# graphdeco-inria/reduced-3dgs

Measured on NVIDIA H100. Metric: rendered Mpixels/s fwd+bwd, higher is better.
Workload: dtype f32

## Files before the change

reduced-3dgs_b200/csrc/gsb_render.cu:

```cuda
#include <cstddef>
#include <cstdlib>
#include "gsb_common.cuh"

namespace gsb {

__device__ __forceinline__ void red_add_v4(float* addr, float a, float b, float c, float d)
{
	asm volatile("red.global.add.v4.f32 [%0], {%1, %2, %3, %4};" ::"l"(addr), "f"(a), "f"(b), "f"(c), "f"(d) : "memory");
}

#define SREC_BYTES 48
__device__ __forceinline__ float4 lds128(uint32_t addr)
{
	float4 v;
	asm volatile("ld.shared.v4.f32 {%0, %1, %2, %3}, [%4];" : "=f"(v.x), "=f"(v.y), "=f"(v.z), "=f"(v.w) : "r"(addr));
	return v;
}
__device__ __forceinline__ float2 lds64(uint32_t addr)
{
	float2 v;
	asm volatile("ld.shared.v2.f32 {%0, %1}, [%2];" : "=f"(v.x), "=f"(v.y) : "r"(addr));
	return v;
}

#define STATS_FIXED_SCALE 68719476736.0f
template <bool STATS, bool MAPS, bool FIXED = false>
__global__ void __launch_bounds__(256, 6) render_forward_kernel(const uint2* __restrict__ ranges,
	const uint32_t* __restrict__ point_list,
	int W, int H, const float4* __restrict__ rec, const float* __restrict__ bg,
	float* __restrict__ final_T, uint32_t* __restrict__ n_contrib, float* __restrict__ out_color, uint32_t* __restrict__ tile_max,
	int32_t* __restrict__ touched_pixels, float* __restrict__ transmittance, float* __restrict__ out_invdepth, float* __restrict__ out_alpha)
{
	__shared__ __align__(16) float4 s_rec[256 * 3];
	__shared__ uint32_t s_id[STATS ? 256 : 1];
	__shared__ uint32_t s_max;
	const int tid = threadIdx.x, lane = tid & 31, warp = tid >> 5;
	const int tile = blockIdx.y * gridDim.x + blockIdx.x;
	const int wx0 = blockIdx.x * GSB_TILE_X + (warp & 1) * 8, wy0 = blockIdx.y * GSB_TILE_Y + (warp >> 1) * 4;
	const int px = wx0 + (lane & 7), py = wy0 + (lane >> 3);
	const bool inside = px < W && py < H;
	const float pxf = (float)px, pyf = (float)py;
	const float rx0 = (float)wx0, rx1 = (float)(wx0 + 7), ry0 = (float)wy0, ry1 = (float)(wy0 + 3);
	const uint2 range = ranges[tile];
	uint32_t sbase = (uint32_t)__cvta_generic_to_shared(s_rec);
	asm volatile("" : "+r"(sbase));
	if (tid == 0) s_max = 0;

	uint32_t Tb = inside ? 0x3f800000u : 0xbf800000u;
	float C0 = 0.0f, C1 = 0.0f, C2 = 0.0f, D = 0.0f;
	uint32_t last = 0;
	for (uint32_t b = range.x; b < range.y; b += 256)
	{
		if (__syncthreads_count((int)Tb < 0) == 256) break;
		const int n = min(256u, range.y - b);
		if (tid < n)
		{
			const uint32_t id = point_list[b + tid];
			const float4 r0 = rec[3 * (size_t)id], r1 = rec[3 * (size_t)id + 1], r2 = rec[3 * (size_t)id + 2];
			s_rec[3 * tid] = r0; s_rec[3 * tid + 1] = r1;
			s_rec[3 * tid + 2] = MAPS ? make_float4(r2.x, r2.y, __fdiv_rn(1.0f, r2.z), r2.w) : r2;
			if (STATS) s_id[tid] = id;
		}
		__syncthreads();
		bool warp_done = __all_sync(0xffffffffu, (int)Tb < 0);
		for (int c0 = 0; c0 < n && !warp_done; c0 += 32)
		{
			const int j = c0 + lane;
			bool keep = false;
			if (j < n)
			{
				const float4 r0 = lds128(sbase + j * SREC_BYTES), r1 = lds128(sbase + j * SREC_BYTES + 16);
				keep = rect_may_contribute(r1.x, r1.y, r0.x, r0.y, r0.z, r0.w, rx0, rx1, ry0, ry1);
			}
			unsigned mask = __ballot_sync(0xffffffffu, keep);
			const uint32_t cbase = sbase + c0 * SREC_BYTES;
			uint32_t nbase = (b - range.x) + c0 + 1;
			asm volatile("" : "+r"(nbase));
			while (mask)
			{
				const int bit = __ffs(mask) - 1; mask &= mask - 1;
				const uint32_t addr = cbase + bit * SREC_BYTES;
				const float4 r0 = lds128(addr), r1 = lds128(addr + 16);
				float2 gb; float invd = 0.0f;
				if (MAPS) { const float4 r2 = lds128(addr + 32); gb = make_float2(r2.x, r2.y); invd = r2.z; }
				else gb = lds64(addr + 32);
				const float T = __uint_as_float(Tb);
				const float dx = __fsub_rn(r1.x, pxf), dy = __fsub_rn(r1.y, pyf);
				const float power = pair_power(r0.x, r0.y, r0.z, dx, dy);
				const bool inwin = !(power > 0.0f) && !(power < r0.w);
				const float alpha = fminf(0.99f, __fmul_rn(r1.z, exp_loop(power)));
				const bool cand = inwin && !(alpha < 1.0f / 255.0f);
				const float test_T = __fmul_rn(T, __fsub_rn(1.0f, alpha));
				const bool stop = cand && (test_T < 0.0001f);
				const bool v = cand && !(test_T < 0.0001f);
				if (STATS)
				{
					const unsigned cm = __ballot_sync(0xffffffffu, v);
					if (cm)
					{
						float ts = v ? T : 0.0f;
#pragma unroll
						for (int o = 16; o > 0; o >>= 1) ts += __shfl_xor_sync(0xffffffffu, ts, o);
						if (lane == 0)
						{
							const uint32_t gid = s_id[c0 + bit];
							atomicAdd(&touched_pixels[gid], (int)__popc(cm));
							if (FIXED) atomicAdd(reinterpret_cast<unsigned long long*>(transmittance) + gid, __float2ull_rn(ts * STATS_FIXED_SCALE));
							else atomicAdd(&transmittance[gid], ts);
						}
					}
				}
				if (v)
				{
					C0 = __fmaf_rn(T, __fmul_rn(r1.w, alpha), C0);
					C1 = __fmaf_rn(T, __fmul_rn(gb.x, alpha), C1);
					C2 = __fmaf_rn(T, __fmul_rn(gb.y, alpha), C2);
					if (MAPS) D = __fmaf_rn(T, __fmul_rn(invd, alpha), D);
					Tb = __float_as_uint(test_T);
					last = nbase + bit;
				}
				if (stop) Tb |= 0x80000000u;
			}
			warp_done = __all_sync(0xffffffffu, (int)Tb < 0);
		}
	}
	const float T = __uint_as_float(Tb & 0x7fffffffu);
	if (inside)
	{
		const size_t pid = (size_t)W * py + px, N = (size_t)W * H;
		final_T[pid] = T;
		n_contrib[pid] = last;
		out_color[pid] = __fmaf_rn(bg[0], T, C0);
		out_color[N + pid] = __fmaf_rn(bg[1], T, C1);
		out_color[2 * N + pid] = __fmaf_rn(bg[2], T, C2);
		if (MAPS) { out_invdepth[pid] = D; out_alpha[pid] = __fsub_rn(1.0f, T); }
	}
	uint32_t m = inside ? last : 0u;
#pragma unroll
	for (int o = 16; o > 0; o >>= 1) m = max(m, __shfl_xor_sync(0xffffffffu, m, o));
	__syncthreads();
	if (lane == 0 && m) atomicMax(&s_max, m);
	__syncthreads();
	if (tid == 0) tile_max[tile] = s_max;
}

#define BWD_BATCH 64
#define STASH_LD 36
#define ACC_STRIDE 9

__device__ __forceinline__ void mma_tf32(float (&d)[4], uint32_t a0, uint32_t a1, uint32_t a2, uint32_t a3, uint32_t b0, uint32_t b1)
{
	asm volatile("mma.sync.aligned.m16n8k8.row.col.f32.tf32.tf32.f32 {%0,%1,%2,%3}, {%4,%5,%6,%7}, {%8,%9}, {%0,%1,%2,%3};"
		: "+f"(d[0]), "+f"(d[1]), "+f"(d[2]), "+f"(d[3]) : "r"(a0), "r"(a1), "r"(a2), "r"(a3), "r"(b0), "r"(b1));
}
__device__ __forceinline__ void split_tf32(float v, uint32_t& hi, uint32_t& lo)
{
	hi = __float_as_uint(v) & 0xffffe000u;
	lo = __float_as_uint(v - __uint_as_float(hi));
}

__device__ __forceinline__ float rcp_approx(float x)
{
	float r;
	asm("rcp.approx.ftz.f32 %0, %1;" : "=f"(r) : "f"(x));
	return r;
}
__device__ __forceinline__ void cp_async16(uint32_t smem_addr, const void* gptr)
{
	asm volatile("cp.async.ca.shared.global [%0], [%1], 16;" ::"r"(smem_addr), "l"(gptr) : "memory");
}
__device__ __forceinline__ void cp_async_commit() { asm volatile("cp.async.commit_group;" ::: "memory"); }
__device__ __forceinline__ void cp_async_wait_all() { asm volatile("cp.async.wait_group 0;" ::: "memory"); }

#define BWD_STAGES 4
template <int NCH> struct BwdWarp {
	float w[16 * STASH_LD];
	float u[16 * STASH_LD];
	float dlp[NCH * 32];
	uint32_t rowid[16];
	uint8_t queue[BWD_BATCH + 16];
};
#define BW_OFF_U (16 * STASH_LD * 4)
#define BW_OFF_ROWID(NCH) (2 * 16 * STASH_LD * 4 + (NCH) * 32 * 4)
#define BW_OFF_QUEUE(NCH) (BW_OFF_ROWID(NCH) + 16 * 4)
template <int NCH> struct BwdSmem {
	float4 rec[BWD_STAGES][BWD_BATCH * 3];
	uint64_t full[BWD_STAGES];
	uint64_t empty[BWD_STAGES];
	float wgt[8 * 32];
	BwdWarp<NCH> wp[8];
};
static_assert(offsetof(BwdWarp<3>, u) == BW_OFF_U && offsetof(BwdWarp<3>, rowid) == BW_OFF_ROWID(3) && offsetof(BwdWarp<3>, queue) == BW_OFF_QUEUE(3), "BwdWarp layout");
static_assert(offsetof(BwdWarp<4>, u) == BW_OFF_U && offsetof(BwdWarp<4>, rowid) == BW_OFF_ROWID(4) && offsetof(BwdWarp<4>, queue) == BW_OFF_QUEUE(4), "BwdWarp layout");
static_assert(sizeof(BwdWarp<3>) % 16 == 0 && sizeof(BwdWarp<4>) % 16 == 0, "BwdWarp alignment");

__device__ __forceinline__ void red_add_v2(float* addr, float a, float b)
{
	asm volatile("red.global.add.v2.f32 [%0], {%1, %2};" ::"l"(addr), "f"(a), "f"(b) : "memory");
}


#define DET_NS(MAPS) ((MAPS) ? 10 : 9)
template <bool MAPS, bool DET = false>
__global__ void __launch_bounds__(256, DET ? 3 : 4) render_backward_kernel(const uint2* __restrict__ ranges,
	const uint32_t* __restrict__ point_list,
	int W, int H, const float4* __restrict__ rec, const float* __restrict__ bg,
	const float* __restrict__ final_Ts, const uint32_t* __restrict__ n_contrib, const uint32_t* __restrict__ tile_max,
	const float* __restrict__ dL_dpixels, float* __restrict__ acc, const float* __restrict__ dL_dinvdepth, const float* __restrict__ dL_dalpha,
	float* __restrict__ parts = nullptr, const uint32_t* __restrict__ slot_offset = nullptr, const uint2* __restrict__ rect = nullptr,
	unsigned long long num_slots = 0)
{
	constexpr int NCH = MAPS ? 4 : 3;
	constexpr int NS = DET_NS(MAPS);
	extern __shared__ __align__(16) unsigned char s_dyn_raw[];
	BwdSmem<NCH>& S = *reinterpret_cast<BwdSmem<NCH>*>(s_dyn_raw);
	float* const ebuf = reinterpret_cast<float*>(s_dyn_raw + sizeof(BwdSmem<NCH>));
	const int tid = threadIdx.x, lane = tid & 31, warp = tid >> 5;
	const int tile = blockIdx.y * gridDim.x + blockIdx.x;
	const uint32_t hi = tile_max[tile];
	if (hi == 0) return;
	const int lx = (warp & 1) * 8 + (lane & 7), ly = (warp >> 1) * 4 + (lane >> 3);
	const int tx0 = blockIdx.x * GSB_TILE_X, ty0 = blockIdx.y * GSB_TILE_Y;
	const int px = tx0 + lx, py = ty0 + ly;
	const bool inside = px < W && py < H;
	const float pxf = (float)px, pyf = (float)py;
	const float rx0 = (float)(tx0 + (warp & 1) * 8), rx1 = rx0 + 7.0f, ry0 = (float)(ty0 + (warp >> 1) * 4), ry1 = ry0 + 3.0f;
	const uint2 range = ranges[tile];
	const size_t pid = (size_t)W * py + px, N = (size_t)W * H;
	uint32_t sbase0 = (uint32_t)__cvta_generic_to_shared(&S.rec[0][0]);
	asm volatile("" : "+r"(sbase0));
	BwdWarp<NCH>& Wp = S.wp[warp];
	uint32_t wbase = (uint32_t)__cvta_generic_to_shared(&Wp);
	asm volatile("" : "+r"(wbase));
	const unsigned lt_mask = (1u << lane) - 1u;

	const float T_final = inside ? final_Ts[pid] : 0.0f;
	float T = T_final;
	const uint32_t last_contributor = inside ? n_contrib[pid] : 0u;
	float dLp0 = 0.f, dLp1 = 0.f, dLp2 = 0.f;
	if (inside) { dLp0 = dL_dpixels[pid]; dLp1 = dL_dpixels[N + pid]; dLp2 = dL_dpixels[2 * N + pid]; }
	float bg_dot_dpixel = bg[0] * dLp0 + bg[1] * dLp1 + bg[2] * dLp2;
	float dLd = 0.f, ar3 = 0.f, lc3 = 0.f;
	if (MAPS && inside)
	{
		if (dL_dinvdepth) dLd = dL_dinvdepth[pid];
		if (dL_dalpha) bg_dot_dpixel -= dL_dalpha[pid];
	}
	float ar0 = 0.f, ar1 = 0.f, ar2 = 0.f, lc0 = 0.f, lc1 = 0.f, lc2 = 0.f, last_alpha = 0.f;
	uint32_t wmax = last_contributor;
#pragma unroll
	for (int o = 16; o > 0; o >>= 1) wmax = max(wmax, __shfl_xor_sync(0xffffffffu, wmax, o));

	const int fg = lane >> 2, ft = lane & 3;
	float* sw = Wp.w;
	float* su = Wp.u;
	uint32_t nrows = 0;
	int buf = 0;

	if (tid < 32)
	{
		const float qx = (float)(tid & 7) - 3.5f, qy = (float)(tid >> 3) - 1.5f;
		S.wgt[0 * 32 + tid] = 1.0f; S.wgt[1 * 32 + tid] = qx; S.wgt[2 * 32 + tid] = qy;
		S.wgt[3 * 32 + tid] = qx * qx; S.wgt[4 * 32 + tid] = qx * qy; S.wgt[5 * 32 + tid] = qy * qy;
		S.wgt[6 * 32 + tid] = 0.0f; S.wgt[7 * 32 + tid] = 0.0f;
	}
	Wp.dlp[lane] = dLp0; Wp.dlp[32 + lane] = dLp1; Wp.dlp[64 + lane] = dLp2;
	if (MAPS) Wp.dlp[96 + lane] = dLd;
	const float cxw = rx0 + 3.5f, cyw = ry0 + 1.5f;
	if (DET) for (int i = tid; i < 8 * BWD_BATCH * NS; i += 256) ebuf[i] = 0.0f;
	__syncthreads();

	auto flush_rows = [&]() {
		if (nrows == 0) return;
		for (uint32_t r = nrows; r < 16; r++) { sw[r * STASH_LD + lane] = 0.f; su[r * STASH_LD + lane] = 0.f; }
		__syncwarp();
		if (!DET && ft == 0)
		{
			if (fg < nrows) asm volatile("prefetch.global.L1 [%0];" ::"l"(rec + 3 * (size_t)Wp.rowid[fg]));
			if (fg + 8 < nrows) asm volatile("prefetch.global.L1 [%0];" ::"l"(rec + 3 * (size_t)Wp.rowid[fg + 8]));
		}
		float dw[4] = { 0.f, 0.f, 0.f, 0.f }, du[4] = { 0.f, 0.f, 0.f, 0.f };
		const float* dl = Wp.dlp + (fg < NCH ? fg : 0) * 32;
#pragma unroll
		for (int kk = 0; kk < 4; kk++)
		{
			const int c0 = 8 * kk + ft, c1 = c0 + 4;
			const uint32_t bw0 = __float_as_uint(S.wgt[fg * 32 + c0]), bw1 = __float_as_uint(S.wgt[fg * 32 + c1]);
			uint32_t buh0, buh1, bul0, bul1;
			split_tf32(fg < NCH ? dl[c0] : 0.0f, buh0, bul0);
			split_tf32(fg < NCH ? dl[c1] : 0.0f, buh1, bul1);
			uint32_t h0, h1, h2, h3, l0, l1, l2, l3;
			split_tf32(sw[fg * STASH_LD + c0], h0, l0); split_tf32(sw[(fg + 8) * STASH_LD + c0], h1, l1);
			split_tf32(sw[fg * STASH_LD + c1], h2, l2); split_tf32(sw[(fg + 8) * STASH_LD + c1], h3, l3);
			mma_tf32(dw, h0, h1, h2, h3, bw0, bw1);
			mma_tf32(dw, l0, l1, l2, l3, bw0, bw1);
			split_tf32(su[fg * STASH_LD + c0], h0, l0); split_tf32(su[(fg + 8) * STASH_LD + c0], h1, l1);
			split_tf32(su[fg * STASH_LD + c1], h2, l2); split_tf32(su[(fg + 8) * STASH_LD + c1], h3, l3);
			mma_tf32(du, h0, h1, h2, h3, buh0, buh1);
			mma_tf32(du, l0, l1, l2, l3, buh0, buh1);
			mma_tf32(du, h0, h1, h2, h3, bul0, bul1);
		}
		const int q1 = (lane & ~3) | 1, q2 = (lane & ~3) | 2;
#pragma unroll
		for (int h = 0; h < 2; h++)
		{
			const float My = __shfl_sync(0xffffffffu, dw[2 * h], q1), Mxx = __shfl_sync(0xffffffffu, dw[2 * h + 1], q1);
			const float Mxy = __shfl_sync(0xffffffffu, dw[2 * h], q2), Myy = __shfl_sync(0xffffffffu, dw[2 * h + 1], q2);
			const float c2 = __shfl_sync(0xffffffffu, du[2 * h], q1);
			float dinvd = 0.f;
			if (MAPS) dinvd = __shfl_sync(0xffffffffu, du[2 * h + 1], q1);
			const uint32_t row = fg + 8 * h;
			if (ft == 0 && row < nrows)
			{
				const uint32_t gid = Wp.rowid[row];
				float4 r0, r1;
				if (DET)
				{
					const uint32_t ra = sbase0 + (uint32_t)(buf * BWD_BATCH * 3) * 16u + gid * SREC_BYTES;
					r0 = lds128(ra); r1 = lds128(ra + 16);
				}
				else { r0 = __ldg(rec + 3 * (size_t)gid); r1 = __ldg(rec + 3 * (size_t)gid + 1); }
				const float X = r1.x - cxw, Y = r1.y - cyw, o = r1.z;
				const float M0 = dw[2 * h], Mx = dw[2 * h + 1];
				const float Sx = X * M0 - Mx, Sy = Y * M0 - My;
				const float Sxx = X * X * M0 - 2.0f * X * Mx + Mxx;
				const float Sxy = X * Y * M0 - X * My - Y * Mx + Mxy;
				const float Syy = Y * Y * M0 - 2.0f * Y * My + Myy;
				if (DET)
				{
					float* e = ebuf + (warp * BWD_BATCH + gid) * NS;
					e[0] = du[2 * h]; e[1] = du[2 * h + 1]; e[2] = c2; e[3] = M0;
					e[4] = -o * (r0.x * Sx + r0.y * Sy); e[5] = -o * (r0.z * Sy + r0.y * Sx); e[6] = o * Sxx; e[7] = o * Sxy;
					e[8] = o * Syy;
					if (MAPS) e[9] = dinvd;
					continue;
				}
				float* a = acc + 12 * (size_t)gid;
				red_add_v4(a, du[2 * h], du[2 * h + 1], c2, M0);
				red_add_v4(a + 4, -o * (r0.x * Sx + r0.y * Sy), -o * (r0.z * Sy + r0.y * Sx), o * Sxx, o * Sxy);
				if (MAPS) red_add_v2(a + 8, o * Syy, dinvd);
				else atomicAdd(a + 8, o * Syy);
			}
		}
		__syncwarp();
		nrows = 0;
	};

	auto list_id = [&](uint32_t bi) -> uint32_t {
		const uint32_t k = bi * BWD_BATCH + tid;
		return (tid < BWD_BATCH && k < hi) ? point_list[range.x + (hi - 1 - k)] : 0xffffffffu;
	};
	auto issue = [&](uint32_t bi, uint32_t id) {
		const int st = bi % BWD_STAGES;
		if (id != 0xffffffffu)
		{
			mbar_arrive_expect_tx(&S.full[st], 48u);
			tma_bulk_g2s(&S.rec[st][3 * tid], rec + 3 * (size_t)id, 48u, &S.full[st]);
		}
		else mbar_arrive(&S.full[st]);
	};
	const uint32_t nb = (hi + BWD_BATCH - 1) / BWD_BATCH;
	if (tid == 0)
	{
		for (int k = 0; k < BWD_STAGES; k++) { mbar_init(&S.full[k], BWD_BATCH); mbar_init(&S.empty[k], 8); }
		mbar_fence_init();
	}
	__syncthreads();
	uint32_t id_next = 0xffffffffu;
	if (tid < BWD_BATCH)
	{
		for (uint32_t k = 0; k < BWD_STAGES - 1 && k < nb; k++) issue(k, list_id(k));
		id_next = list_id(BWD_STAGES - 1);
	}
	for (uint32_t bi = 0; bi < nb; bi++)
	{
		const uint32_t b = bi * BWD_BATCH;
		const int n = min((uint32_t)BWD_BATCH, hi - b);
		buf = bi % BWD_STAGES;
		if (tid < BWD_BATCH && bi + BWD_STAGES - 1 < nb)
		{
			if (bi >= 1) mbar_wait(&S.empty[(bi - 1) % BWD_STAGES], ((bi - 1) / BWD_STAGES) & 1u);
			issue(bi + BWD_STAGES - 1, id_next);
			id_next = list_id(bi + BWD_STAGES);
		}
		mbar_wait(&S.full[buf], (bi / BWD_STAGES) & 1u);
		const uint32_t sbase = sbase0 + (uint32_t)(buf * BWD_BATCH * 3) * 16u;
		uint32_t qn = 0;
		for (int c0 = 0; c0 < n; c0 += 32)
		{
			const int j = c0 + lane;
			bool keep = false;
			if (j < n && (hi - 1 - b - j) < wmax)
			{
				const float4 r0 = lds128(sbase + j * SREC_BYTES), r1 = lds128(sbase + j * SREC_BYTES + 16);
				keep = rect_may_contribute(r1.x, r1.y, r0.x, r0.y, r0.z, r0.w, rx0, rx1, ry0, ry1);
			}
			const unsigned mask = __ballot_sync(0xffffffffu, keep);
			if (keep) Wp.queue[qn + __popc(mask & lt_mask)] = (uint8_t)j;
			qn += __popc(mask);
		}
		__syncwarp();
		uint32_t posb = hi - 1 - b;
		asm volatile("" : "+r"(posb));
		uint32_t jj = 0, jnext;
		if (qn) asm volatile("ld.shared.u8 %0, [%1+%2];" : "=r"(jj) : "r"(wbase), "n"(BW_OFF_QUEUE(NCH)));
		for (uint32_t q = 0; q < qn; q++, jj = jnext)
		{
			asm volatile("ld.shared.u8 %0, [%1+%2];" : "=r"(jnext) : "r"(wbase + q), "n"(BW_OFF_QUEUE(NCH) + 1));
			const uint32_t pos = posb - jj;
			const uint32_t addr = sbase + jj * SREC_BYTES;
			const float4 r0 = lds128(addr), r1 = lds128(addr + 16);
			const float dx = __fsub_rn(r1.x, pxf), dy = __fsub_rn(r1.y, pyf);
			const float power = pair_power(r0.x, r0.y, r0.z, dx, dy);
			const float G = exp_loop(power);
			const float alpha = fminf(0.99f, __fmul_rn(r1.z, G));
			const bool active = (pos < last_contributor) && !(power > 0.0f) && !(power < r0.w) && !(alpha < 1.0f / 255.0f);
			if (!__any_sync(0xffffffffu, active)) continue;
			float wv = 0.f, uv = 0.f;
			const float4 r2 = lds128(addr + 32);
			if (active)
			{
				const float inv = rcp_approx(1.0f - alpha);
				T = T * inv;
				uv = alpha * T;
				const float cr = r1.w, cg = r2.x, cb = r2.y;
				const float oml = 1.0f - last_alpha;
				ar0 = last_alpha * lc0 + oml * ar0; lc0 = cr;
				ar1 = last_alpha * lc1 + oml * ar1; lc1 = cg;
				ar2 = last_alpha * lc2 + oml * ar2; lc2 = cb;
				float dL_dalpha = (cr - ar0) * dLp0 + (cg - ar1) * dLp1 + (cb - ar2) * dLp2;
				if (MAPS)
				{
					const float invd = rcp_approx(r2.z);
					float dLd_p;
					asm volatile("ld.shared.f32 %0, [%1+%2];" : "=f"(dLd_p) : "r"(wbase + lane * 4), "n"(2 * 16 * STASH_LD * 4 + 96 * 4));
					ar3 = last_alpha * lc3 + oml * ar3; lc3 = invd;
					dL_dalpha += (invd - ar3) * dLd_p;
				}
				dL_dalpha *= T;
				last_alpha = alpha;
				dL_dalpha += (-T_final * inv) * bg_dot_dpixel;
				wv = G * dL_dalpha;
			}
			{
				const uint32_t sa = wbase + (nrows * STASH_LD + lane) * 4;
				asm volatile("st.shared.f32 [%0], %1;" ::"r"(sa), "f"(wv) : "memory");
				asm volatile("st.shared.f32 [%0+%2], %1;" ::"r"(sa), "f"(uv), "n"(BW_OFF_U) : "memory");
				if (lane == 0) asm volatile("st.shared.f32 [%0+%2], %1;" ::"r"(wbase + nrows * 4), "f"(DET ? __uint_as_float(jj) : r2.w), "n"(BW_OFF_ROWID(NCH)) : "memory");
			}
			nrows++;
			if (nrows == 16) flush_rows();
		}
		if (DET)
		{
			flush_rows();
			__syncthreads();
			const int j = tid >> 2;
			if (j < n)
			{
				const uint32_t gid = __float_as_uint(S.rec[buf][3 * j + 2].w);
				const uint2 rc = rect[gid];
				const uint32_t minx = rc.x & 0xffffu, maxx = rc.x >> 16, miny = rc.y & 0xffffu;
				const unsigned long long slot = (unsigned long long)slot_offset[gid] + (blockIdx.y - miny) * (maxx - minx) + (blockIdx.x - minx);
				for (int k = tid & 3; k < NS; k += 4)
				{
					float s = ebuf[j * NS + k];
					ebuf[j * NS + k] = 0.0f;
#pragma unroll
					for (int w = 1; w < 8; w++)
					{
						s += ebuf[(w * BWD_BATCH + j) * NS + k];
						ebuf[(w * BWD_BATCH + j) * NS + k] = 0.0f;
					}
					if (slot < num_slots) parts[slot * NS + k] = s;
				}
			}
			__syncthreads();
		}
		__syncwarp();
		if (lane == 0) mbar_arrive(&S.empty[buf]);
	}
	flush_rows();
}

__global__ void __launch_bounds__(256) stats_fixed_to_float_kernel(int P, const unsigned long long* __restrict__ fixed, float* __restrict__ out)
{
	const int i = blockIdx.x * blockDim.x + threadIdx.x;
	if (i < P) out[i] = __fmul_rn(__ull2float_rn(fixed[i]), 1.0f / STATS_FIXED_SCALE);
}

int launch_stats_fixed_to_float(int P, const unsigned long long* fixed, float* out, cudaStream_t stream)
{
	if (P <= 0) return GSB_OK;
	ProfScope prof(K_TOOLS, stream);
	stats_fixed_to_float_kernel<<<(P + 255) / 256, 256, 0, stream>>>(P, fixed, out);
	GSB_LAUNCHED();
	GSB_CUDA_OK(cudaGetLastError());
	return GSB_OK;
}

int launch_render_forward(const ForwardRequest& req, const ImageState& img, const BinningState& b, const GeomState& g)
{
	const int W = req.cam->width, H = req.cam->height;
	const dim3 grid((W + GSB_TILE_X - 1) / GSB_TILE_X, (H + GSB_TILE_Y - 1) / GSB_TILE_Y);
	const bool fixed = req.touched_pixels && req.transmittance_fixed;
	const bool stats = fixed || (req.touched_pixels && req.transmittance);
	const bool maps = !stats && req.out_invdepth && req.out_alpha;
	float* const transmittance = fixed ? reinterpret_cast<float*>(req.transmittance_fixed) : req.transmittance;
	ProfScope prof(K_RENDER_FWD, req.stream);
	return dispatch([&](auto stats, auto maps, auto fixed) -> int {
		if constexpr (!(stats && maps) && (stats || !fixed))
			render_forward_kernel<stats, maps, fixed><<<grid, 256, 0, req.stream>>>(img.ranges, b.point_list, W, H, g.rec,
				req.cam->background, img.final_T, img.n_contrib, req.out_color, img.tile_max_contrib, stats ? req.touched_pixels : nullptr,
				stats ? transmittance : nullptr, maps ? req.out_invdepth : nullptr, maps ? req.out_alpha : nullptr);
		GSB_LAUNCHED();
		GSB_CUDA_OK(cudaGetLastError());
		return GSB_OK;
	}, stats, maps, fixed);
}

int launch_render_backward(const BackwardRequest& req, const ImageState& img, const BinningState& b, const GeomState& g, float* acc,
	float* parts, const uint32_t* slot_offset)
{
	const int W = req.cam->width, H = req.cam->height;
	const dim3 grid((W + GSB_TILE_X - 1) / GSB_TILE_X, (H + GSB_TILE_Y - 1) / GSB_TILE_Y);
	const cudaStream_t stream = req.stream;
	return dispatch([&](auto maps, auto det) -> int {
		const size_t smem = sizeof(BwdSmem<maps ? 4 : 3>) + (det ? size_t(8) * BWD_BATCH * DET_NS(maps) * sizeof(float) : 0);
		auto kernel = render_backward_kernel<maps, det>;
		if (int e = ensure_dyn_smem((const void*)kernel, (int)smem)) return e;
		if (det)
		{
			ProfScope prof(K_DET_CLEAR, stream);
			GSB_CUDA_OK(cudaMemsetAsync(parts, 0, size_t(req.R) * DET_NS(maps) * sizeof(float), stream));
		}
		ProfScope prof(K_RENDER_BWD, stream);
		if (!det) GSB_CUDA_OK(cudaMemsetAsync(acc, 0, size_t(req.scene->P) * 48, stream));
		kernel<<<grid, 256, smem, stream>>>(img.ranges, b.point_list, W, H, g.rec, req.cam->background,
			img.final_T, img.n_contrib, img.tile_max_contrib, req.dL_dout_color, det ? nullptr : acc, req.dL_dinvdepth, req.dL_dalpha,
			parts, slot_offset, det ? g.rect : nullptr, det ? (unsigned long long)req.R : 0ull);
		GSB_LAUNCHED();
		GSB_CUDA_OK(cudaGetLastError());
		return GSB_OK;
	}, req.dL_dinvdepth || req.dL_dalpha, req.deterministic);
}

}
```

Baseline: 579.9.

## Stash per-row Gaussian constants in shared memory and transpose MMA results for flush

The backward flush no longer reloads each Gaussian record from global memory (or prefetches it into L1). Lane 0 instead stores the record's conic, mean and opacity into spare columns of the per-warp stash rows when the row is produced. The MMA outputs are written back to shared memory so that one lane per row reads its moments with vector loads, replacing the shuffle-based gather. The B-fragment weights and dL/dpixel vectors are pre-permuted so each lane loads them with two float4 loads. The row counter is also kept as a byte offset. This relies on STASH_LD leaving room past column 32 and adds extra shared stores and syncwarps per flush.

```diff
diff --git a/reduced-3dgs_b200/csrc/gsb_render.cu b/reduced-3dgs_b200/csrc/gsb_render.cu
--- a/reduced-3dgs_b200/csrc/gsb_render.cu
+++ b/reduced-3dgs_b200/csrc/gsb_render.cu
@@ -177,12 +177,13 @@
 	float w[16 * STASH_LD];
 	float u[16 * STASH_LD];
 	float dlp[NCH * 32];
-	uint32_t rowid[16];
 	uint8_t queue[BWD_BATCH + 16];
 };
 #define BW_OFF_U (16 * STASH_LD * 4)
-#define BW_OFF_ROWID(NCH) (2 * 16 * STASH_LD * 4 + (NCH) * 32 * 4)
-#define BW_OFF_QUEUE(NCH) (BW_OFF_ROWID(NCH) + 16 * 4)
+#define BW_OFF_CONST (32 * 4)
+#define BW_OFF_DLP (2 * 16 * STASH_LD * 4)
+#define BW_OFF_QUEUE(NCH) (BW_OFF_DLP + (NCH) * 32 * 4)
+__device__ __forceinline__ int bwd_frag_slot(int p) { return (p & 3) * 8 + 2 * (p >> 3) + ((p >> 2) & 1); }
 template <int NCH> struct BwdSmem {
 	float4 rec[BWD_STAGES][BWD_BATCH * 3];
 	uint64_t full[BWD_STAGES];
@@ -190,8 +191,9 @@
 	float wgt[8 * 32];
 	BwdWarp<NCH> wp[8];
 };
-static_assert(offsetof(BwdWarp<3>, u) == BW_OFF_U && offsetof(BwdWarp<3>, rowid) == BW_OFF_ROWID(3) && offsetof(BwdWarp<3>, queue) == BW_OFF_QUEUE(3), "BwdWarp layout");
-static_assert(offsetof(BwdWarp<4>, u) == BW_OFF_U && offsetof(BwdWarp<4>, rowid) == BW_OFF_ROWID(4) && offsetof(BwdWarp<4>, queue) == BW_OFF_QUEUE(4), "BwdWarp layout");
+static_assert(offsetof(BwdWarp<3>, u) == BW_OFF_U && offsetof(BwdWarp<3>, dlp) == BW_OFF_DLP && offsetof(BwdWarp<3>, queue) == BW_OFF_QUEUE(3), "BwdWarp layout");
+static_assert(offsetof(BwdWarp<4>, u) == BW_OFF_U && offsetof(BwdWarp<4>, dlp) == BW_OFF_DLP && offsetof(BwdWarp<4>, queue) == BW_OFF_QUEUE(4), "BwdWarp layout");
+static_assert(offsetof(BwdSmem<3>, wp) % 16 == 0 && offsetof(BwdSmem<4>, wp) % 16 == 0 && offsetof(BwdSmem<3>, wgt) % 16 == 0, "BwdSmem alignment");
 static_assert(sizeof(BwdWarp<3>) % 16 == 0 && sizeof(BwdWarp<4>) % 16 == 0, "BwdWarp alignment");
 
 __device__ __forceinline__ void red_add_v2(float* addr, float a, float b)
@@ -233,6 +235,7 @@
 	uint32_t wbase = (uint32_t)__cvta_generic_to_shared(&Wp);
 	asm volatile("" : "+r"(wbase));
 	const unsigned lt_mask = (1u << lane) - 1u;
+	const uint32_t wlane = wbase + lane * 4;
 
 	const float T_final = inside ? final_Ts[pid] : 0.0f;
 	float T = T_final;
@@ -254,41 +257,40 @@
 	const int fg = lane >> 2, ft = lane & 3;
 	float* sw = Wp.w;
 	float* su = Wp.u;
-	uint32_t nrows = 0;
+	uint32_t srow = 0;
 	int buf = 0;
 
-	if (tid < 32)
-	{
-		const float qx = (float)(tid & 7) - 3.5f, qy = (float)(tid >> 3) - 1.5f;
-		S.wgt[0 * 32 + tid] = 1.0f; S.wgt[1 * 32 + tid] = qx; S.wgt[2 * 32 + tid] = qy;
-		S.wgt[3 * 32 + tid] = qx * qx; S.wgt[4 * 32 + tid] = qx * qy; S.wgt[5 * 32 + tid] = qy * qy;
-		S.wgt[6 * 32 + tid] = 0.0f; S.wgt[7 * 32 + tid] = 0.0f;
-	}
-	Wp.dlp[lane] = dLp0; Wp.dlp[32 + lane] = dLp1; Wp.dlp[64 + lane] = dLp2;
-	if (MAPS) Wp.dlp[96 + lane] = dLd;
+	{
+		const int k = 8 * ((tid >> 1) & 3) + ((tid >> 3) & 3) + 4 * (tid & 1), n = tid >> 5;
+		const float qx = (float)(k & 7) - 3.5f, qy = (float)(k >> 3) - 1.5f;
+		S.wgt[tid] = n == 0 ? 1.0f : n == 1 ? qx : n == 2 ? qy : n == 3 ? qx * qx : n == 4 ? qx * qy : n == 5 ? qy * qy : 0.0f;
+	}
+	const int fslot = bwd_frag_slot(lane);
+	Wp.dlp[fslot] = dLp0; Wp.dlp[32 + fslot] = dLp1; Wp.dlp[64 + fslot] = dLp2;
+	if (MAPS) Wp.dlp[96 + fslot] = dLd;
 	const float cxw = rx0 + 3.5f, cyw = ry0 + 1.5f;
 	if (DET) for (int i = tid; i < 8 * BWD_BATCH * NS; i += 256) ebuf[i] = 0.0f;
 	__syncthreads();
 
 	auto flush_rows = [&]() {
-		if (nrows == 0) return;
+		if (srow == 0) return;
+		const uint32_t nrows = srow / (STASH_LD * 4);
 		for (uint32_t r = nrows; r < 16; r++) { sw[r * STASH_LD + lane] = 0.f; su[r * STASH_LD + lane] = 0.f; }
 		__syncwarp();
-		if (!DET && ft == 0)
-		{
-			if (fg < nrows) asm volatile("prefetch.global.L1 [%0];" ::"l"(rec + 3 * (size_t)Wp.rowid[fg]));
-			if (fg + 8 < nrows) asm volatile("prefetch.global.L1 [%0];" ::"l"(rec + 3 * (size_t)Wp.rowid[fg + 8]));
-		}
 		float dw[4] = { 0.f, 0.f, 0.f, 0.f }, du[4] = { 0.f, 0.f, 0.f, 0.f };
-		const float* dl = Wp.dlp + (fg < NCH ? fg : 0) * 32;
+		const float4 bwa = reinterpret_cast<const float4*>(S.wgt)[2 * lane], bwb = reinterpret_cast<const float4*>(S.wgt)[2 * lane + 1];
+		float4 bua = make_float4(0.f, 0.f, 0.f, 0.f), bub = bua;
+		if (fg < NCH) { bua = reinterpret_cast<const float4*>(Wp.dlp)[2 * lane]; bub = reinterpret_cast<const float4*>(Wp.dlp)[2 * lane + 1]; }
+		const float bwv[8] = { bwa.x, bwa.y, bwa.z, bwa.w, bwb.x, bwb.y, bwb.z, bwb.w };
+		const float buv[8] = { bua.x, bua.y, bua.z, bua.w, bub.x, bub.y, bub.z, bub.w };
 #pragma unroll
 		for (int kk = 0; kk < 4; kk++)
 		{
 			const int c0 = 8 * kk + ft, c1 = c0 + 4;
-			const uint32_t bw0 = __float_as_uint(S.wgt[fg * 32 + c0]), bw1 = __float_as_uint(S.wgt[fg * 32 + c1]);
+			const uint32_t bw0 = __float_as_uint(bwv[2 * kk]), bw1 = __float_as_uint(bwv[2 * kk + 1]);
 			uint32_t buh0, buh1, bul0, bul1;
-			split_tf32(fg < NCH ? dl[c0] : 0.0f, buh0, bul0);
-			split_tf32(fg < NCH ? dl[c1] : 0.0f, buh1, bul1);
+			split_tf32(buv[2 * kk], buh0, bul0);
+			split_tf32(buv[2 * kk + 1], buh1, bul1);
 			uint32_t h0, h1, h2, h3, l0, l1, l2, l3;
 			split_tf32(sw[fg * STASH_LD + c0], h0, l0); split_tf32(sw[(fg + 8) * STASH_LD + c0], h1, l1);
 			split_tf32(sw[fg * STASH_LD + c1], h2, l2); split_tf32(sw[(fg + 8) * STASH_LD + c1], h3, l3);
@@ -300,50 +302,45 @@
 			mma_tf32(du, l0, l1, l2, l3, buh0, buh1);
 			mma_tf32(du, h0, h1, h2, h3, bul0, bul1);
 		}
-		const int q1 = (lane & ~3) | 1, q2 = (lane & ~3) | 2;
-#pragma unroll
-		for (int h = 0; h < 2; h++)
-		{
-			const float My = __shfl_sync(0xffffffffu, dw[2 * h], q1), Mxx = __shfl_sync(0xffffffffu, dw[2 * h + 1], q1);
-			const float Mxy = __shfl_sync(0xffffffffu, dw[2 * h], q2), Myy = __shfl_sync(0xffffffffu, dw[2 * h + 1], q2);
-			const float c2 = __shfl_sync(0xffffffffu, du[2 * h], q1);
-			float dinvd = 0.f;
-			if (MAPS) dinvd = __shfl_sync(0xffffffffu, du[2 * h + 1], q1);
-			const uint32_t row = fg + 8 * h;
-			if (ft == 0 && row < nrows)
-			{
-				const uint32_t gid = Wp.rowid[row];
-				float4 r0, r1;
-				if (DET)
-				{
-					const uint32_t ra = sbase0 + (uint32_t)(buf * BWD_BATCH * 3) * 16u + gid * SREC_BYTES;
-					r0 = lds128(ra); r1 = lds128(ra + 16);
-				}
-				else { r0 = __ldg(rec + 3 * (size_t)gid); r1 = __ldg(rec + 3 * (size_t)gid + 1); }
-				const float X = r1.x - cxw, Y = r1.y - cyw, o = r1.z;
-				const float M0 = dw[2 * h], Mx = dw[2 * h + 1];
-				const float Sx = X * M0 - Mx, Sy = Y * M0 - My;
-				const float Sxx = X * X * M0 - 2.0f * X * Mx + Mxx;
-				const float Sxy = X * Y * M0 - X * My - Y * Mx + Mxy;
-				const float Syy = Y * Y * M0 - 2.0f * Y * My + Myy;
-				if (DET)
-				{
-					float* e = ebuf + (warp * BWD_BATCH + gid) * NS;
-					e[0] = du[2 * h]; e[1] = du[2 * h + 1]; e[2] = c2; e[3] = M0;
-					e[4] = -o * (r0.x * Sx + r0.y * Sy); e[5] = -o * (r0.z * Sy + r0.y * Sx); e[6] = o * Sxx; e[7] = o * Sxy;
-					e[8] = o * Syy;
-					if (MAPS) e[9] = dinvd;
-					continue;
-				}
+		__syncwarp();
+		*reinterpret_cast<float2*>(&sw[fg * STASH_LD + 2 * ft]) = make_float2(dw[0], dw[1]);
+		*reinterpret_cast<float2*>(&sw[(fg + 8) * STASH_LD + 2 * ft]) = make_float2(dw[2], dw[3]);
+		*reinterpret_cast<float2*>(&su[fg * STASH_LD + 2 * ft]) = make_float2(du[0], du[1]);
+		*reinterpret_cast<float2*>(&su[(fg + 8) * STASH_LD + 2 * ft]) = make_float2(du[2], du[3]);
+		__syncwarp();
+		if (lane < nrows)
+		{
+			const float4 mw = *reinterpret_cast<const float4*>(&sw[lane * STASH_LD]);
+			const float2 mw2 = *reinterpret_cast<const float2*>(&sw[lane * STASH_LD + 4]);
+			const float4 cu = *reinterpret_cast<const float4*>(&su[lane * STASH_LD]);
+			const float4 cn = *reinterpret_cast<const float4*>(&sw[lane * STASH_LD + 32]);
+			const float4 mo = *reinterpret_cast<const float4*>(&su[lane * STASH_LD + 32]);
+			const uint32_t gid = __float_as_uint(cn.w);
+			const float X = mo.x - cxw, Y = mo.y - cyw, o = mo.z;
+			const float M0 = mw.x, Mx = mw.y, My = mw.z, Mxx = mw.w, Mxy = mw2.x, Myy = mw2.y;
+			const float Sx = X * M0 - Mx, Sy = Y * M0 - My;
+			const float Sxx = X * X * M0 - 2.0f * X * Mx + Mxx;
+			const float Sxy = X * Y * M0 - X * My - Y * Mx + Mxy;
+			const float Syy = Y * Y * M0 - 2.0f * Y * My + Myy;
+			if (DET)
+			{
+				float* e = ebuf + (warp * BWD_BATCH + gid) * NS;
+				e[0] = cu.x; e[1] = cu.y; e[2] = cu.z; e[3] = M0;
+				e[4] = -o * (cn.x * Sx + cn.y * Sy); e[5] = -o * (cn.z * Sy + cn.y * Sx); e[6] = o * Sxx; e[7] = o * Sxy;
+				e[8] = o * Syy;
+				if (MAPS) e[9] = cu.w;
+			}
+			else
+			{
 				float* a = acc + 12 * (size_t)gid;
-				red_add_v4(a, du[2 * h], du[2 * h + 1], c2, M0);
-				red_add_v4(a + 4, -o * (r0.x * Sx + r0.y * Sy), -o * (r0.z * Sy + r0.y * Sx), o * Sxx, o * Sxy);
-				if (MAPS) red_add_v2(a + 8, o * Syy, dinvd);
+				red_add_v4(a, cu.x, cu.y, cu.z, M0);
+				red_add_v4(a + 4, -o * (cn.x * Sx + cn.y * Sy), -o * (cn.z * Sy + cn.y * Sx), o * Sxx, o * Sxy);
+				if (MAPS) red_add_v2(a + 8, o * Syy, cu.w);
 				else atomicAdd(a + 8, o * Syy);
 			}
 		}
 		__syncwarp();
-		nrows = 0;
+		srow = 0;
 	};
 
 	auto list_id = [&](uint32_t bi) -> uint32_t {
@@ -433,7 +430,7 @@
 				{
 					const float invd = rcp_approx(r2.z);
 					float dLd_p;
-					asm volatile("ld.shared.f32 %0, [%1+%2];" : "=f"(dLd_p) : "r"(wbase + lane * 4), "n"(2 * 16 * STASH_LD * 4 + 96 * 4));
+					asm volatile("ld.shared.f32 %0, [%1+%2];" : "=f"(dLd_p) : "r"(wbase + fslot * 4), "n"(BW_OFF_DLP + 96 * 4));
 					ar3 = last_alpha * lc3 + oml * ar3; lc3 = invd;
 					dL_dalpha += (invd - ar3) * dLd_p;
 				}
@@ -443,13 +440,19 @@
 				wv = G * dL_dalpha;
 			}
 			{
-				const uint32_t sa = wbase + (nrows * STASH_LD + lane) * 4;
+				const uint32_t sa = wlane + srow;
 				asm volatile("st.shared.f32 [%0], %1;" ::"r"(sa), "f"(wv) : "memory");
 				asm volatile("st.shared.f32 [%0+%2], %1;" ::"r"(sa), "f"(uv), "n"(BW_OFF_U) : "memory");
-				if (lane == 0) asm volatile("st.shared.f32 [%0+%2], %1;" ::"r"(wbase + nrows * 4), "f"(DET ? __uint_as_float(jj) : r2.w), "n"(BW_OFF_ROWID(NCH)) : "memory");
-			}
-			nrows++;
-			if (nrows == 16) flush_rows();
+				if (lane == 0)
+				{
+					asm volatile("st.shared.v4.f32 [%0+%5], {%1, %2, %3, %4};" ::"r"(sa), "f"(r0.x), "f"(r0.y), "f"(r0.z),
+						"f"(DET ? __uint_as_float(jj) : r2.w), "n"(BW_OFF_CONST) : "memory");
+					asm volatile("st.shared.v4.f32 [%0+%5], {%1, %2, %3, %4};" ::"r"(sa), "f"(r1.x), "f"(r1.y), "f"(r1.z), "f"(r1.w),
+						"n"(BW_OFF_U + BW_OFF_CONST) : "memory");
+				}
+			}
+			srow += STASH_LD * 4;
+			if (srow == 16 * STASH_LD * 4) flush_rows();
 		}
 		if (DET)
 		{
```

Result: faster. 594.6 (median of 6 runs) (+2.5%).
